# ferreiraluisa/implementation-phd-lab-vision

Hardware: AMD Instinct MI355X
Metric: H36M frames/sec ResNet-50 feature extraction (higher is better)
Workload: dtype bf16; 1 GPU; ResNet-50[:-1] bf16 forward, batch 256 x 224x224x3 fp32 NCHW frames per GPU (BASELINE configs[1]), seeded synthetic weights, (N,2048) fp32 features; batch_per_gpu=256, micro_batch=0, lanes=2, lanes_requested=2, lanes_mode=2 lanes (1.066 x one lane), input=f32, parallelism=frames sharded over 1 rank(s)

## Files before the change

### implementation_phd_lab_vision_amd/csrc/kernels.h

```cpp
#pragma once
#include <hip/hip_runtime.h>
#include <stdint.h>
#include <type_traits>

typedef __attribute__((ext_vector_type(8))) __bf16 bf16x8;
typedef __attribute__((ext_vector_type(4))) float f32x4;
typedef __attribute__((ext_vector_type(4))) unsigned int u32x4;
typedef __attribute__((ext_vector_type(2))) unsigned int u32x2;

#define GLOBAL_AS __attribute__((address_space(1)))
#define LDS_AS __attribute__((address_space(3)))

__device__ __forceinline__ float bf16_bits_to_f32(unsigned int hi16) { return __uint_as_float(hi16 << 16); }

__device__ __forceinline__ unsigned int pack_bf16x2(float lo, float hi) {
    typedef __attribute__((ext_vector_type(2))) __bf16 bf16x2;
    typedef __attribute__((ext_vector_type(2))) float f32x2;
    f32x2 v = {lo, hi};
    bf16x2 b = __builtin_convertvector(v, bf16x2);
    return __builtin_bit_cast(unsigned int, b);
}

typedef __attribute__((ext_vector_type(8))) _Float16 f16x8;
typedef __attribute__((ext_vector_type(2))) _Float16 f16x2;
// ... 561 lines not shown
        unsigned y_voff = 0u;
        constexpr unsigned ESZ = (ET == 2) ? 1u : 2u;
        const unsigned y_rowstep = (unsigned)(16 * a.y_cstride) * ESZ;

        f32x4 bias_reg[MR];
        auto bias_fetch = [&](int tile) {
            const int pt = (int)fast_div((unsigned)tile, a.div_ctiles);
            const int c0 = (tile - pt * a.n_ctiles) * BC;
#pragma unroll
            for (int t = 0; t < MR / 2; ++t) {
                bias_reg[2 * t] = *reinterpret_cast<const f32x4*>(a.bias + c0 + cout_lane + 32 * t);
                bias_reg[2 * t + 1] = *reinterpret_cast<const f32x4*>(a.bias + c0 + cout_lane + 32 * t + 4);
            }
        };
        auto tile_begin = [&]() {
            const int pt = (int)fast_div((unsigned)c_tile, a.div_ctiles);
            const int c0 = (c_tile - pt * a.n_ctiles) * BC, p0 = pt * BP;
            y_voff = (unsigned)((p0 + pix_lane) * a.y_cstride + c0 + cout_lane) * ESZ;
#pragma unroll
            for (int t = 0; t < MR / 2; ++t) {
                const f32x4 b_lo = bias_reg[2 * t];
                const f32x4 b_hi = bias_reg[2 * t + 1];
#pragma unroll
                for (int j = 0; j < NR; ++j) {
                    acc[2 * t][j] = b_lo;
                    acc[2 * t + 1][j] = b_hi;
                    if constexpr (PREFETCH_RES) if (has_res) {
                        if constexpr (ET == 2) {
                            const u32x2 r2 = __builtin_amdgcn_raw_buffer_load_b64(rsrc_r, y_voff + j * y_rowstep + 32 * t, 0, 0);
                            res_reg[t][j] = (u32x4){r2[0], r2[1], 0u, 0u};
                        } else {
                            res_reg[t][j] = __builtin_amdgcn_raw_buffer_load_b128(rsrc_r, y_voff + j * y_rowstep + 64 * t, 0, 0);
                        }
                    }
                }
            }
        };
        auto compute = [&]() {
            const char* sbase = smem + c_buf * STAGE_BYTES;
            bf16x8 wf[2][MR], xf[2][NR];
#pragma unroll
            for (int kk = 0; kk < 2; ++kk) {
                const int ph = fphys0 ^ (kk << 6);
#pragma unroll
                for (int j = 0; j < NR; ++j) xf[kk][j] = *reinterpret_cast<const bf16x8*>(sbase + x_frag + j * 2048 + ph);
#pragma unroll
                for (int m = 0; m < MR; ++m) wf[kk][m] = *reinterpret_cast<const bf16x8*>(sbase + w_frag + m * 2048 + ph);
            }
            if constexpr (ET == 2) {
#pragma unroll
                for (int m = 0; m < MR; ++m)
#pragma unroll
                    for (int j = 0; j < NR; ++j) acc[m][j] = mfma_fp8_k128(wf[0][m], wf[1][m], xf[0][j], xf[1][j], acc[m][j]);
            } else {
#pragma unroll
            for (int kk = 0; kk < 2; ++kk)
#pragma unroll
                for (int m = 0; m < MR; ++m)
#pragma unroll
                    for (int j = 0; j < NR; ++j)
                        acc[m][j] = mfma_e<ET>(wf[kk][m], xf[kk][j], acc[m][j]);
            }
            if constexpr (NCONS + NLOAD <= 8 && ET != 2) {
                __builtin_amdgcn_sched_group_barrier(0x100, 2 * (MR + NR), 0);
                __builtin_amdgcn_sched_group_barrier(0x008, 2 * MR * NR, 0);
            }
        };
        auto epilogue = [&]() {
#pragma unroll
            for (int t = 0; t < MR / 2; ++t) {
#pragma unroll
                for (int j = 0; j < NR; ++j) {
                    f32x4 lo = acc[2 * t][j], hi = acc[2 * t + 1][j];
                    const unsigned voff = y_voff + j * y_rowstep + 32 * ESZ * t;
                    if constexpr (ET == 2) {
#pragma unroll
                        for (int e = 0; e < 4; ++e) { lo[e] *= a.oscale; hi[e] *= a.oscale; }
                        if (has_res) {
                            u32x2 r;
                            if constexpr (PREFETCH_RES) r = (u32x2){res_reg[t][j][0], res_reg[t][j][1]};
                            else r = __builtin_amdgcn_raw_buffer_load_b64(rsrc_r, voff, 0, 0);
                            lo[0] += __builtin_amdgcn_cvt_f32_fp8((int)r[0], 0) * a.rscale; lo[1] += __builtin_amdgcn_cvt_f32_fp8((int)r[0], 1) * a.rscale;
                            lo[2] += __builtin_amdgcn_cvt_f32_fp8((int)r[0], 2) * a.rscale; lo[3] += __builtin_amdgcn_cvt_f32_fp8((int)r[0], 3) * a.rscale;
                            hi[0] += __builtin_amdgcn_cvt_f32_fp8((int)r[1], 0) * a.rscale; hi[1] += __builtin_amdgcn_cvt_f32_fp8((int)r[1], 1) * a.rscale;
                            hi[2] += __builtin_amdgcn_cvt_f32_fp8((int)r[1], 2) * a.rscale; hi[3] += __builtin_amdgcn_cvt_f32_fp8((int)r[1], 3) * a.rscale;
                        }
                        if (a.relu) {
#pragma unroll
                            for (int e = 0; e < 4; ++e) { lo[e] = fmaxf(lo[e], 0.f); hi[e] = fmaxf(hi[e], 0.f); }
                        }
                        const u32x2 o8 = (u32x2){pack4_fp8(lo[0], lo[1], lo[2], lo[3]), pack4_fp8(hi[0], hi[1], hi[2], hi[3])};
                        __builtin_amdgcn_raw_buffer_store_b64(o8, rsrc_y, voff, 0, 0);
                        continue;
                    }
                    if (has_res) {
                        u32x4 r;
                        if constexpr (PREFETCH_RES) r = res_reg[t][j];
                        else r = __builtin_amdgcn_raw_buffer_load_b128(rsrc_r, voff, 0, 0);
                        lo[0] += unpack_lo_e<ET>(r[0]); lo[1] += unpack_hi_e<ET>(r[0]);
                        lo[2] += unpack_lo_e<ET>(r[1]); lo[3] += unpack_hi_e<ET>(r[1]);
                        hi[0] += unpack_lo_e<ET>(r[2]); hi[1] += unpack_hi_e<ET>(r[2]);
                        hi[2] += unpack_lo_e<ET>(r[3]); hi[3] += unpack_hi_e<ET>(r[3]);
                    }
                    u32x4 out = (u32x4){pack2_e<ET>(lo[0], lo[1]), pack2_e<ET>(lo[2], lo[3]), pack2_e<ET>(hi[0], hi[1]),
                                        pack2_e<ET>(hi[2], hi[3])};
                    if (a.relu) {
#pragma unroll
                        for (int e = 0; e < 4; ++e) out[e] = relu_bf16x2(out[e]);
                    }
                    if constexpr (ET != 2) {
                        if (a.q_inv > 0.f) {
                            const u32x2 o8 = (u32x2){
                                pack4_fp8(unpack_lo_e<ET>(out[0]) * a.q_inv, unpack_hi_e<ET>(out[0]) * a.q_inv, unpack_lo_e<ET>(out[1]) * a.q_inv, unpack_hi_e<ET>(out[1]) * a.q_inv),
                                pack4_fp8(unpack_lo_e<ET>(out[2]) * a.q_inv, unpack_hi_e<ET>(out[2]) * a.q_inv, unpack_lo_e<ET>(out[3]) * a.q_inv, unpack_hi_e<ET>(out[3]) * a.q_inv)};
                            __builtin_amdgcn_raw_buffer_store_b64(o8, rsrc_y, voff >> 1, 0, 0);
                            continue;
                        }
                    }
                    __builtin_amdgcn_raw_buffer_store_b128(out, rsrc_y, voff, 0, 0);
                }
            }
        };
        if (total > 0) bias_fetch(c_tile);
        __builtin_amdgcn_s_barrier();
        R50_STAMP_DECL
        for (int g = 0; g < total; ++g) {
            if (c_k == 0) tile_begin();
            R50_MARK(0)
            compute();
#if defined(R50_STAMP)
            __builtin_amdgcn_sched_barrier(0);
            asm volatile("s_nop 0" ::"v"(acc[MR - 1][NR - 1]) : "memory");
#endif
            R50_MARK(1)
            c_buf = (c_buf == NSTAGE - 1) ? 0 : c_buf + 1;
            if (++c_k == a.nk) {
                const int next_tile = c_tile + grid;
                if (next_tile < a.n_blocks) bias_fetch(next_tile);
                epilogue();
                c_k = 0;
                c_tile = next_tile;
            }
            R50_MARK(2)
            __builtin_amdgcn_s_barrier();
            R50_MARK(3)
        }
        R50_STAMP_FLUSH(NCONS + NLOAD)
    }
#else
    (void)a;
#endif
}

template <int ET, int NR, bool DUAL>
__global__ __launch_bounds__(512) void gemm8p_kernel(const ConvArgs a) {
#if defined(__HIP_DEVICE_COMPILE__)
    static_assert(NR == 8 || NR == 7, "pixel blocks per wave: 8 (256-pixel tile) or 7 (224)");
    constexpr int BC = 256, BP = 32 * NR;
    constexpr int NA1 = NR - 4;
    constexpr int SLOT = 16384, KBUF = 4 * SLOT;
    extern __shared__ __attribute__((aligned(16))) char smem[];

    const int tid = threadIdx.x;
    const int lane = tid & 63;
    const int wave = __builtin_amdgcn_readfirstlane(tid >> 6);
    const int wr = wave >> 2, wc = wave & 3;
    const int fr = lane & 15, fq = lane >> 4;
    const int srow = tid >> 3;
    const int lchunk = (tid & 7) ^ (srow & 7);

    const int grid = gridDim.x;
    const int first = xcd_remap(blockIdx.x, grid);
    const int my_tiles = (a.n_blocks - first + grid - 1) / grid;
    const int total = my_tiles * a.nk;

    const __amdgpu_buffer_rsrc_t rsrc_w = __builtin_amdgcn_make_buffer_rsrc(const_cast<__bf16*>(a.w), 0, a.w_bytes, 0x00020000);
    const __amdgpu_buffer_rsrc_t rsrc_x = __builtin_amdgcn_make_buffer_rsrc(const_cast<__bf16*>(a.x), 0, a.x_records, 0x00020000);
    const __amdgpu_buffer_rsrc_t rsrc_x2 = __builtin_amdgcn_make_buffer_rsrc(const_cast<__bf16*>(DUAL ? a.x2 : a.x), 0, DUAL ? a.x2_records : 0u, 0x00020000);
    const __amdgpu_buffer_rsrc_t rsrc_y = __builtin_amdgcn_make_buffer_rsrc(a.y, 0, a.y_bytes, 0x00020000);
    const __amdgpu_buffer_rsrc_t rsrc_r = __builtin_amdgcn_make_buffer_rsrc(const_cast<__bf16*>(a.res), 0, a.res ? a.y_bytes : 0u, 0x00020000);

    unsigned w_voff[2][2], x_voff[2][2], x2_voff[DUAL ? 2 : 1][2];
#pragma unroll
    for (int s = 0; s < 2; ++s)
#pragma unroll
        for (int i = 0; i < 2; ++i) {
            const int q5 = srow & 31;
            const int cl = 128 * i + 64 * (srow >> 5) + 32 * s + ((q5 & 3) | (((q5 >> 4) & 1) << 2) | (((q5 >> 2) & 3) << 3));
            w_voff[s][i] = (unsigned)(cl * a.Ktot + lchunk * 8) * 2u;
        }
    int s_tile = first, s_kt = 0, s_buf = 0, s_rem = total, s_wbase = 0;
    auto decode_tile = [&](int tile) {
        const int pt = (int)fast_div((unsigned)tile, a.div_ctiles);
        const int p0 = pt * BP;
        s_wbase = (tile - pt * a.n_ctiles) * BC * a.Ktot * 2;
#pragma unroll
        for (int s = 0; s < 2; ++s)
#pragma unroll
            for (int i = 0; i < 2; ++i) {
                const int m = p0 + 16 * NR * i + 64 * s + srow;
                unsigned v = kOobOffset, v2 = kOobOffset;
                if ((s == 0 || srow < 16 * NA1) && m < a.M) {
                    const int n = (int)fast_div((unsigned)m, a.div_howo);
                    const int r = m - n * a.HoWo;
                    const int ho = (int)fast_div((unsigned)r, a.div_wo);
                    const int wo = r - ho * a.Wo;
                    v = (unsigned)(((n * a.H + ho * a.stride) * a.W + wo * a.stride) * a.x_cstride + lchunk * 8) * 2u;
                    if constexpr (DUAL) v2 = (unsigned)(((n * a.H2 + ho * a.stride2) * a.W2 + wo * a.stride2) * a.x2_cstride + lchunk * 8) * 2u;
                }
                x_voff[s][i] = v;
                if constexpr (DUAL) x2_voff[s][i] = v2;
            }
    };
    auto stage = [&](auto slot_c) {
        constexpr int SL = decltype(slot_c)::value;
        if (s_rem > 0) {
            char* dst = smem + s_buf * KBUF + SL * SLOT + wave * 1024;
            if constexpr ((SL & 1) == 0) {
                const int soff = __builtin_amdgcn_readfirstlane(s_wbase + s_kt * 128);
#pragma unroll
                for (int i = 0; i < 2; ++i)
                    __builtin_amdgcn_raw_ptr_buffer_load_lds(rsrc_w, (LDS_AS void*)(dst + i * 8192), 16, w_voff[SL >> 1][i], soff, 0, 0);
            } else {
                const bool second = DUAL && s_kt >= a.cc1;
                const int soff = __builtin_amdgcn_readfirstlane((second ? s_kt - a.cc1 : s_kt) * 128);
                const __amdgpu_buffer_rsrc_t rs = second ? rsrc_x2 : rsrc_x;
#pragma unroll
                for (int i = 0; i < 2; ++i) {
                    const unsigned v = second ? x2_voff[DUAL ? (SL >> 1) : 0][i] : x_voff[SL >> 1][i];
                    __builtin_amdgcn_raw_ptr_buffer_load_lds(rs, (LDS_AS void*)(dst + i * 8192), 16, v, soff, 0, 0);
                }
            }
            if constexpr (SL == 3) {
                --s_rem;
                s_buf ^= 1;
                if (++s_kt == a.nk) {
                    s_kt = 0;
                    s_tile += grid;
                    if (s_tile < a.n_blocks) decode_tile(s_tile);
                }
            }
        }
    };
    using std::integral_constant;

    f32x4 acc[4][NR];
    f32x4 bias_reg[4];
    const bool has_res = (a.res != nullptr);
    const int fphys0 = (fq ^ (fr & 7)) << 4;
    const int w_fr[2] = {(32 * wc + fr) * 128 + fphys0, (32 * wc + fr) * 128 + (fphys0 ^ 64)};
    const int x_fr[2] = {SLOT + (64 * wr + fr) * 128 + fphys0, SLOT + (64 * wr + fr) * 128 + (fphys0 ^ 64)};
    const int cout_lane = 64 * wc + 8 * fq;
    const int pix_lane = 16 * NR * wr + fr;
    int c_tile = first, c_kt = 0;
    unsigned y_voff = 0u;
    const unsigned y_rowstep = (unsigned)(16 * a.y_cstride * 2);
    auto bias_fetch = [&](int tile) {
        const int pt = (int)fast_div((unsigned)tile, a.div_ctiles);
        const int c0 = (tile - pt * a.n_ctiles) * BC;
#pragma unroll
        for (int t = 0; t < 2; ++t) {
            bias_reg[2 * t] = *reinterpret_cast<const f32x4*>(a.bias + c0 + cout_lane + 32 * t);
            bias_reg[2 * t + 1] = *reinterpret_cast<const f32x4*>(a.bias + c0 + cout_lane + 32 * t + 4);
        }
    };
    auto tile_begin = [&]() {
        const int pt = (int)fast_div((unsigned)c_tile, a.div_ctiles);
        const int c0 = (c_tile - pt * a.n_ctiles) * BC, p0 = pt * BP;
        y_voff = (unsigned)((p0 + pix_lane) * a.y_cstride + c0 + cout_lane) * 2u;
#pragma unroll
        for (int m = 0; m < 4; ++m)
#pragma unroll
            for (int j = 0; j < NR; ++j) acc[m][j] = bias_reg[m];
    };
    auto epilogue = [&]() {
#pragma unroll
        for (int j = 0; j < NR; ++j) {
            u32x4 rres[2];
            if (has_res) {
#pragma unroll
                for (int t = 0; t < 2; ++t) rres[t] = __builtin_amdgcn_raw_buffer_load_b128(rsrc_r, y_voff + j * y_rowstep + 64 * t, 0, 0);
            }
#pragma unroll
            for (int t = 0; t < 2; ++t) {
                f32x4 lo = acc[2 * t][j], hi = acc[2 * t + 1][j];
                if (has_res) {
                    const u32x4 r = rres[t];
                    lo[0] += unpack_lo_e<ET>(r[0]); lo[1] += unpack_hi_e<ET>(r[0]);
                    lo[2] += unpack_lo_e<ET>(r[1]); lo[3] += unpack_hi_e<ET>(r[1]);
                    hi[0] += unpack_lo_e<ET>(r[2]); hi[1] += unpack_hi_e<ET>(r[2]);
                    hi[2] += unpack_lo_e<ET>(r[3]); hi[3] += unpack_hi_e<ET>(r[3]);
                }
                u32x4 out = (u32x4){pack2_e<ET>(lo[0], lo[1]), pack2_e<ET>(lo[2], lo[3]), pack2_e<ET>(hi[0], hi[1]), pack2_e<ET>(hi[2], hi[3])};
                if (a.relu) {
#pragma unroll
                    for (int e = 0; e < 4; ++e) out[e] = relu_bf16x2(out[e]);
                }
                __builtin_amdgcn_raw_buffer_store_b128(out, rsrc_y, y_voff + j * y_rowstep + 64 * t, 0, 0);
            }
        }
    };
#define G8_BARRIER() { __builtin_amdgcn_sched_barrier(0); __builtin_amdgcn_s_barrier(); __builtin_amdgcn_sched_barrier(0); }
#define G8_LGKM(n) { asm volatile("s_waitcnt lgkmcnt(" #n ")" ::: "memory"); __builtin_amdgcn_sched_barrier(0); }
#define G8_PRIO_UP() __builtin_amdgcn_s_setprio(1)
#define G8_PRIO_DN() __builtin_amdgcn_s_setprio(0)

    if (total > 0) {
        bias_fetch(c_tile);
        decode_tile(s_tile);
        stage(integral_constant<int, 0>{}); stage(integral_constant<int, 1>{}); stage(integral_constant<int, 2>{}); stage(integral_constant<int, 3>{});
        stage(integral_constant<int, 0>{}); stage(integral_constant<int, 1>{}); stage(integral_constant<int, 2>{});
        if (total >= 2) {
            asm volatile("s_waitcnt vmcnt(6)" ::: "memory");
        } else {
            asm volatile("s_waitcnt vmcnt(0)" ::: "memory");
        }
    }
    G8_BARRIER();
    if (wr == 1) G8_BARRIER();

    bf16x8 xf[4][2], wf0[2][2], wf1[2][2];
    for (int g = 0; g < total; ++g) {
        const char* kb = smem + (g & 1) * KBUF;
        if (c_kt == 0) tile_begin();
#pragma unroll
        for (int m = 0; m < 2; ++m)
#pragma unroll
            for (int kk = 0; kk < 2; ++kk) wf0[m][kk] = *reinterpret_cast<const bf16x8*>(kb + w_fr[kk] + m * 2048);
        __builtin_amdgcn_sched_barrier(0);
#pragma unroll
        for (int j = 0; j < 4; ++j)
#pragma unroll
            for (int kk = 0; kk < 2; ++kk) xf[j][kk] = *reinterpret_cast<const bf16x8*>(kb + x_fr[kk] + j * 2048);
        __builtin_amdgcn_sched_barrier(0);
        stage(integral_constant<int, 3>{});
        G8_LGKM(8)
        G8_BARRIER();
        G8_LGKM(0)
        G8_PRIO_UP();
#pragma unroll
        for (int kk = 0; kk < 2; ++kk)
#pragma unroll
            for (int m = 0; m < 2; ++m)
#pragma unroll
                for (int j = 0; j < 4; ++j) acc[m][j] = mfma_e<ET>(wf0[m][kk], xf[j][kk], acc[m][j]);
        G8_PRIO_DN();
        G8_BARRIER();
#pragma unroll
        for (int m = 0; m < 2; ++m)
#pragma unroll
            for (int kk = 0; kk < 2; ++kk) wf1[m][kk] = *reinterpret_cast<const bf16x8*>(kb + 2 * SLOT + w_fr[kk] + m * 2048);
        __builtin_amdgcn_sched_barrier(0);
        stage(integral_constant<int, 0>{});
        G8_BARRIER();
        G8_LGKM(0)
        G8_PRIO_UP();
#pragma unroll
        for (int kk = 0; kk < 2; ++kk)
#pragma unroll
            for (int m = 0; m < 2; ++m)
#pragma unroll
                for (int j = 0; j < 4; ++j) acc[2 + m][j] = mfma_e<ET>(wf1[m][kk], xf[j][kk], acc[2 + m][j]);
        G8_PRIO_DN();
        G8_BARRIER();
#pragma unroll
        for (int j = 0; j < NA1; ++j)
#pragma unroll
            for (int kk = 0; kk < 2; ++kk) xf[j][kk] = *reinterpret_cast<const bf16x8*>(kb + 2 * SLOT + x_fr[kk] + j * 2048);
        __builtin_amdgcn_sched_barrier(0);
        stage(integral_constant<int, 1>{});
        G8_BARRIER();
        G8_LGKM(0)
        G8_PRIO_UP();
#pragma unroll
        for (int kk = 0; kk < 2; ++kk)
#pragma unroll
            for (int m = 0; m < 2; ++m)
#pragma unroll
                for (int j = 0; j < NA1; ++j) acc[2 + m][4 + j] = mfma_e<ET>(wf1[m][kk], xf[j][kk], acc[2 + m][4 + j]);
        G8_PRIO_DN();
        G8_BARRIER();
        stage(integral_constant<int, 2>{});
        if (g + 2 < total) {
            asm volatile("s_waitcnt vmcnt(6)" ::: "memory");
        } else {
            asm volatile("s_waitcnt vmcnt(0)" ::: "memory");
        }
        G8_BARRIER();
        G8_PRIO_UP();
#pragma unroll
        for (int kk = 0; kk < 2; ++kk)
#pragma unroll
            for (int m = 0; m < 2; ++m)
#pragma unroll
                for (int j = 0; j < NA1; ++j) acc[m][4 + j] = mfma_e<ET>(wf0[m][kk], xf[j][kk], acc[m][4 + j]);
        G8_PRIO_DN();
        G8_BARRIER();
        if (++c_kt == a.nk) {
            const int next_tile = c_tile + grid;
            if (next_tile < a.n_blocks) bias_fetch(next_tile);
            epilogue();
            c_kt = 0;
            c_tile = next_tile;
        }
    }
    if (wr == 0) G8_BARRIER();
#undef G8_BARRIER
#undef G8_LGKM
#undef G8_PRIO_UP
#undef G8_PRIO_DN
#else
    (void)a;
#endif
}

template <int ET>
__global__ __launch_bounds__(512) void conv3x3_c64_kernel(const ConvArgs a) {
#if defined(__HIP_DEVICE_COMPILE__)
    constexpr int W_BYTES = 9 * 64 * 128;
    constexpr int XROWS_LDS = 352;
    constexpr int X_BYTES = XROWS_LDS * 128;
    constexpr int NPASS = 11;
    extern __shared__ __attribute__((aligned(16))) char smem[];
    const int tid = threadIdx.x, lane = tid & 63;
    const int wave = __builtin_amdgcn_readfirstlane(tid >> 6);

    for (int i = tid; i < 9 * 64 * 8; i += 512) {
        const int c = i & 7, rho = (i >> 3) & 63, tap = i >> 9;
        const int cl = (rho & ~31) | (rho & 3) | (((rho >> 4) & 1) << 2) | (((rho >> 2) & 3) << 3);
        *reinterpret_cast<u32x4*>(smem + tap * 8192 + rho * 128 + ((c ^ (rho & 7)) << 4)) =
            *reinterpret_cast<const u32x4*>(a.w + (size_t)cl * 576 + tap * 64 + c * 8);
    }
    const int grid = gridDim.x;
    const int n_tiles = a.N * 14;
    const int first = blockIdx.x;
    const int my_tiles = (n_tiles - first + grid - 1) / grid;

    if (wave >= 4) {
        const int lw = wave - 4;
        const __amdgpu_buffer_rsrc_t rsrc_x = __builtin_amdgcn_make_buffer_rsrc(
            const_cast<char*>(reinterpret_cast<const char*>(a.x) - a.x_back), 0, a.x_records, 0x00020000);
        unsigned rel[NPASS];
        unsigned top_mask = 0u, bot_mask = 0u, ok_mask = 0u;
#pragma unroll
        for (int i = 0; i < NPASS; ++i) {
            const int rho = i * 32 + lw * 8 + (lane >> 3);
            const int rr = rho / 58, col = rho - rr * 58;
            const int chunk = (lane & 7) ^ (col & 7);
            rel[i] = (unsigned)((rr * 56 + col) * 128 + chunk * 16);
            if (rho < 348 && col >= 1 && col <= 56) ok_mask |= 1u << i;
            if (rr == 0) top_mask |= 1u << i;
            if (rr == 5) bot_mask |= 1u << i;
        }
        auto issue = [&](int tile, int buf) {
            const int n = tile / 14, tr = tile - n * 14;
            const unsigned base = (unsigned)((n * 56 + tr * 4) * 56) * 128u;
            unsigned valid = ok_mask;
            if (tr == 0) valid &= ~top_mask;
            if (tr == 13) valid &= ~bot_mask;
            char* dst = smem + W_BYTES + buf * X_BYTES + lw * 1024;
#pragma unroll
            for (int i = 0; i < NPASS; ++i) {
                const unsigned voff = ((valid >> i) & 1u) ? base + rel[i] : kOobOffset;
                __builtin_amdgcn_raw_ptr_buffer_load_lds(rsrc_x, (LDS_AS void*)(dst + i * 4096), 16, voff, 0, 0, 0);
            }
        };
        if (my_tiles > 0) issue(first, 0);
        __syncthreads();
        for (int t = 0; t < my_tiles; ++t) {
            asm volatile("s_waitcnt vmcnt(0)" ::: "memory");
            __builtin_amdgcn_s_barrier();
            if (t + 1 < my_tiles) issue(first + (t + 1) * grid, (t + 1) & 1);
        }
    } else {
        const int wave_c = wave >> 1, wave_p = wave & 1;
        const int fr = lane & 15, fq = lane >> 4;
        const __amdgpu_buffer_rsrc_t rsrc_y = __builtin_amdgcn_make_buffer_rsrc(a.y, 0, a.y_bytes, 0x00020000);
        const int cout_lane = wave_c * 32 + 8 * fq;
        const f32x4 b_lo = *reinterpret_cast<const f32x4*>(a.bias + cout_lane);
        const f32x4 b_hi = *reinterpret_cast<const f32x4*>(a.bias + cout_lane + 4);
        const int w_frag = (wave_c * 32 + fr) * 128 + ((fq ^ (fr & 7)) << 4);
        int xa[7][3];
#pragma unroll
        for (int j = 0; j < 7; ++j) {
            const int p = wave_p * 112 + 16 * j + fr;
            const int r = p / 56, c = p - r * 56;
#pragma unroll
            for (int kw = 0; kw < 3; ++kw) xa[j][kw] = (r * 58 + c + kw) * 128 + ((fq ^ ((c + kw) & 7)) << 4);
        }
        __syncthreads();
        for (int t = 0; t < my_tiles; ++t) {
            __builtin_amdgcn_s_barrier();
            const char* xb = smem + W_BYTES + (t & 1) * X_BYTES;
            f32x4 acc[2][7];
#pragma unroll
            for (int j = 0; j < 7; ++j) { acc[0][j] = b_lo; acc[1][j] = b_hi; }
            bf16x8 wf[2][2], xf[2][7];
            auto read_block = [&](int it, bf16x8 (&w)[2], bf16x8 (&x)[7]) {
                const int tap = it >> 1, kk = it & 1, kh = tap / 3, kw = tap - kh * 3;
                const char* wt = smem + tap * 8192;
                w[0] = *reinterpret_cast<const bf16x8*>(wt + (w_frag ^ (kk << 6)));
                w[1] = *reinterpret_cast<const bf16x8*>(wt + 2048 + (w_frag ^ (kk << 6)));
#pragma unroll
                for (int j = 0; j < 7; ++j)
                    x[j] = *reinterpret_cast<const bf16x8*>(xb + kh * (58 * 128) + (xa[j][kw] ^ (kk << 6)));
            };
            read_block(0, wf[0], xf[0]);
#pragma unroll
            for (int it = 0; it < 18; ++it) {
                if (it + 1 < 18) read_block(it + 1, wf[(it + 1) & 1], xf[(it + 1) & 1]);
#pragma unroll
                for (int j = 0; j < 7; ++j) {
                    acc[0][j] = mfma_e<ET>(wf[it & 1][0], xf[it & 1][j], acc[0][j]);
                    acc[1][j] = mfma_e<ET>(wf[it & 1][1], xf[it & 1][j], acc[1][j]);
                }
                if (it + 1 < 18) __builtin_amdgcn_sched_group_barrier(0x100, 9, 0);
                __builtin_amdgcn_sched_group_barrier(0x008, 14, 0);
            }
            const int tile = first + t * grid;
            const unsigned pix0 = (unsigned)(tile * 224 + wave_p * 112 + fr);
#pragma unroll
            for (int j = 0; j < 7; ++j) {
                const f32x4 lo = acc[0][j], hi = acc[1][j];
                u32x4 o = (u32x4){pack2_e<ET>(lo[0], lo[1]), pack2_e<ET>(lo[2], lo[3]), pack2_e<ET>(hi[0], hi[1]),
                                  pack2_e<ET>(hi[2], hi[3])};
                if (a.relu) {
#pragma unroll
                    for (int e = 0; e < 4; ++e) o[e] = relu_bf16x2(o[e]);
                }
                __builtin_amdgcn_raw_buffer_store_b128(o, rsrc_y, (pix0 + 16 * j) * 128u + cout_lane * 2, 0, 0);
            }
        }
    }
#else
    (void)a;
#endif
}

template <int ET, int NI, int TR, int IW, int IH>
__global__ __launch_bounds__(768) void conv3x3_xres_kernel(const ConvArgs a) {
#if defined(__HIP_DEVICE_COMPILE__)
    constexpr int BC = 128, TPS = 1, NST = 3, SCHED = 0, RB = 1;
    constexpr bool RB7 = RB && IW == 7;
    static_assert(RB == 0 || (TPS == 1 && (NST == 3 || RB == 1) && SCHED == 0 && ((NI == 1 && (IW == 14 || IW == 28) && TR * (IW == 14 ? 16 : 32) == 224) || (NI == 4 && IW == 7 && TR == 7 && RB == 1))),
                  "row blocks: 14 blocks of 16 positions");
    static_assert(RB != 3 || BC == 128, "32-wide blocks: four consumer waves of 32 couts");
    constexpr int NCW = RB == 3 ? 4 : 8;
    constexpr int PW = RB ? (IW == 28 ? 32 : 16) : IW + 2, PP = (TR + 2) * PW, PPT = RB7 ? 17 * 16 : NI * PP;
    constexpr int BSTEP = RB7 ? 8 : 7;
    constexpr int XPASS = (PPT + 31) / 32, XBUF = XPASS * 32 * 128;
    constexpr int NPX = NI * TR * IW, NBLK = RB ? 14 : (NPX + 15) / 16;
    static_assert(RB || NBLK == 13, "tiles are 196 pixels");
// ... 4981 lines not shown
```

### implementation_phd_lab_vision_amd/csrc/r50_abi.hip

```cpp
#include "kernels.h"
#include "smooth_kernels.h"
#include "multiview_kernels.h"
#include "kinematics_kernels.h"
#include "refine_kernels.h"
#include "track_kernels.h"
#include "resample_kernels.h"
#include "bootstrap_kernels.h"
#include "launch_plan.h"
#include "../../include/r50.h"
#include "../../include/r50_hal.h"
#include "../../include/r50_smooth.h"
#include "../../include/r50_multiview.h"
#include "../../include/r50_kinematics.h"
#include "../../include/r50_refine.h"
#include "../../include/r50_track.h"
#include "../../include/r50_resample.h"
#include "../../include/r50_bootstrap.h"

#include <atomic>
#include <cmath>
#include <cstdlib>
#include <cstdio>
#include <cstring>
#include <initializer_list>
// ... 294 lines not shown
                    out[(((size_t)kh * 64 + rho) * 8 + (kw + 1)) * 4 + c] = part == 2 ? f32_to_f16_rne(w) : part ? f32_to_bf16_rne(w - bf16_to_f32(hd)) : hd;
                }
        }
}

FastDiv make_fast_div(unsigned d) {
    FastDiv f{0u, 0u};
    if (d <= 1u) return f;
    unsigned L = 0;
    while ((1ull << L) < d) ++L;
    f.shr = L - 1;
    const unsigned long long num = 1ull << (32 + f.shr);
    f.mul = (unsigned)((num + d - 1) / d);
    return f;
}

constexpr int kPersistBit = 32;
int g_num_cus = 0;
int g_cu_cap = [] { const char* v = std::getenv("R50_CU_CAP"); return v ? std::atoi(v) : 0; }();
int cu_budget(int device_cus) { return (g_cu_cap > 0 && g_cu_cap < device_cus) ? g_cu_cap : device_cus; }
int num_cus() {
    if (g_num_cus == 0) {
        int dev = 0;
        hipDeviceProp_t prop;
        if (hipGetDevice(&dev) != hipSuccess || hipGetDeviceProperties(&prop, dev) != hipSuccess) return 0;
        g_num_cus = cu_budget(prop.multiProcessorCount);
    }
    return g_num_cus;
}

template <typename K, typename... Args>
Launch launch_persistent(K kern, long long tiles, int threads, size_t lds, hipStream_t s, Args... args) {
    const hipError_t e = hipFuncSetAttribute(reinterpret_cast<const void*>(kern), hipFuncAttributeMaxDynamicSharedMemorySize, (int)lds);
    if (e != hipSuccess) return e;
    const int cus = num_cus();
    if (cus == 0) return hipErrorInvalidDevice;
    hipLaunchKernelGGL(kern, dim3((unsigned)(tiles < cus ? tiles : cus)), dim3(threads), lds, s, args...);
    return hipGetLastError();
}

template <int ET, int BC, int BP, int WC, int WP, int NSTAGE, bool SPLIT = false>
Launch launch_igemm_t(ConvArgs a, bool persistent, hipStream_t s) {
    a.n_ctiles = a.Cout / BC;
    a.n_blocks = a.n_ctiles * ((a.M + BP - 1) / BP);
    a.div_ctiles = make_fast_div((unsigned)a.n_ctiles);
    constexpr int kRowsPerPass = WC * WP * 8;
    const size_t lds = (size_t)NSTAGE * (BC + (BP + kRowsPerPass - 1) / kRowsPerPass * kRowsPerPass) * 128;
    auto kern = igemm_bf16_kernel<ET, BC, BP, WC, WP, NSTAGE, SPLIT>;
    if (lds > 65536) {
        hipError_t e = hipFuncSetAttribute(reinterpret_cast<const void*>(kern),
                                           hipFuncAttributeMaxDynamicSharedMemorySize, (int)lds);
        if (e != hipSuccess) return e;
    }
    int grid = a.n_blocks;
    if (persistent) {
        const int cus = num_cus();
        if (cus == 0) return hipErrorInvalidDevice;
        static int per_cu = 0;
        if (per_cu == 0) {
            int n = 0;
            if (hipOccupancyMaxActiveBlocksPerMultiprocessor(&n, kern, WC * WP * 64, lds) != hipSuccess || n < 1) n = 1;
            per_cu = n;
        }
        if (grid > cus * per_cu) grid = cus * per_cu;
    }
    hipLaunchKernelGGL(kern, dim3(grid), dim3(WC * WP * 64), lds, s, a);
    return hipGetLastError();
}

struct TunedTile { int h, cin, cout, ks, stride, res, tile; };
constexpr TunedTile kTuned[] = {
    {56, 64, 64, 1, 1, 0, 73},    {56, 64, 64, 3, 1, 0, 2},     {56, 64, 256, 1, 1, 1, 72},   {56, 64, 256, 1, 1, 0, 38},
    {56, 256, 64, 1, 1, 0, 73},    {56, 256, 128, 1, 1, 0, 40},  {56, 128, 128, 3, 2, 0, 65},   {28, 128, 512, 1, 1, 1, 72},
    {56, 256, 512, 1, 2, 0, 42},  {28, 512, 128, 1, 1, 0, 65},   {28, 128, 128, 3, 1, 0, 72},  {28, 512, 256, 1, 1, 0, 72},
    {28, 256, 256, 3, 2, 0, 44},  {14, 256, 1024, 1, 1, 1, 72}, {28, 512, 1024, 1, 2, 0, 72}, {14, 1024, 256, 1, 1, 0, 44},
    {14, 256, 256, 3, 1, 0, 68},  {14, 1024, 512, 1, 1, 0, 72}, {14, 512, 512, 3, 2, 0, 68},  {7, 512, 2048, 1, 1, 1, 43},
    {14, 1024, 2048, 1, 2, 0, 43}, {7, 2048, 512, 1, 1, 0, 72}, {7, 512, 512, 3, 1, 0, 68},
};

constexpr int kWsBit = 64;

template <int ET, int BC, int BP, int CWC, int CWP, int NLOAD, int NSTAGE>
Launch launch_igemm_ws_t(ConvArgs a, hipStream_t s) {
    a.n_ctiles = a.Cout / BC;
    a.n_blocks = a.n_ctiles * ((a.M + BP - 1) / BP);
    a.div_ctiles = make_fast_div((unsigned)a.n_ctiles);
    constexpr int kRowsPerPass = NLOAD * 8;
    const size_t lds = (size_t)NSTAGE * (BC + (BP + kRowsPerPass - 1) / kRowsPerPass * kRowsPerPass) * 128;
    return launch_persistent(igemm_ws_kernel<ET, BC, BP, CWC, CWP, NLOAD, NSTAGE>, a.n_blocks, (CWC * CWP + NLOAD) * 64, lds, s, a);
}

constexpr int kTileC64 = kWsBit | 16;
bool is_c64_shape(const ConvArgs& a) {
    return a.ks == 3 && a.stride == 1 && a.pad == 1 && a.Cin == 64 && a.Cout == 64 && a.H == 56 && a.W == 56 && a.res == nullptr &&
           a.x_cstride == 64 && a.y_cstride == 64 && a.Ktot == 576;
}
template <int ET>
Launch launch_conv3x3_c64(const ConvArgs& a, hipStream_t s) {
    if (!is_c64_shape(a)) return Launch::refused();
    constexpr size_t lds = 9 * 64 * 128 + 2 * 352 * 128;
    return launch_persistent(conv3x3_c64_kernel<ET>, a.N * 14, 512, lds, s, a);
}

constexpr int kTileXres = kWsBit | 17;
bool is_xres_shape(const ConvArgs& a) {
    if (!(a.ks == 3 && a.stride == 1 && a.pad == 1 && a.Cin == a.Cout && a.H == a.W && a.res == nullptr && a.x2 == nullptr &&
          a.x_cstride == a.Cin && a.y_cstride == a.Cout && a.Ktot == 9 * a.Cin && a.et != 2)) return false;
    return (a.H == 14 && a.Cin == 256) || (a.H == 7 && a.Cin == 512) || (a.H == 28 && a.Cin == 128);
}
template <int ET, int NI, int TR, int IW, int IH>
Launch launch_conv3x3_xres_t(ConvArgs a, hipStream_t s) {
    constexpr int BC = 128, NST = 3;
    constexpr int PW = IW == 28 ? 32 : 16;
    constexpr int PPT = IW == 7 ? 17 * 16 : NI * (TR + 2) * PW, XBUF = (PPT + 31) / 32 * 32 * 128;
    constexpr size_t lds = 2 * (size_t)XBUF + NST * (size_t)BC * 128;
    static_assert(lds <= 163840, "LDS budget");
    a.n_ctiles = a.Cout / BC;
    a.n_blocks = ((a.N + NI - 1) / NI) * (IH / TR) * a.n_ctiles;
    return launch_persistent(conv3x3_xres_kernel<ET, NI, TR, IW, IH>, a.n_blocks, 768, lds, s, a);
}
template <int ET>
Launch launch_conv3x3_xres(const ConvArgs& a, hipStream_t s) {
    if (!is_xres_shape(a)) return Launch::refused();
    if (a.H == 14) return launch_conv3x3_xres_t<ET, 1, 14, 14, 14>(a, s);
    if (a.H == 28) return launch_conv3x3_xres_t<ET, 1, 7, 28, 28>(a, s);
    return launch_conv3x3_xres_t<ET, 4, 7, 7, 7>(a, s);
}

constexpr int kTileS2 = kWsBit | 18;
bool is_s2_shape(const ConvArgs& a) {
    if (!(a.ks == 3 && a.stride == 2 && a.pad == 1 && a.Cin == a.Cout && a.H == a.W && a.res == nullptr && a.x2 == nullptr &&
          a.x_cstride == a.Cin && a.y_cstride == a.Cout && a.Ktot == 9 * a.Cin && a.et != 2)) return false;
    return (a.H == 56 && a.Cin == 128) || (a.H == 28 && a.Cin == 256) || (a.H == 14 && a.Cin == 512);
}
template <int ET, int TR, int OW, int OH>
Launch launch_conv3x3_s2_t(ConvArgs a, hipStream_t s) {
    constexpr size_t lds = 3 * 32768 + 3 * 128 * 128;
    a.n_ctiles = a.Cout / 128;
    a.n_blocks = (OW == 7 ? (a.N + 3) / 4 : a.N * (OH / TR)) * a.n_ctiles;
    return launch_persistent(conv3x3_s2_kernel<ET, 128, TR, OW, OH>, a.n_blocks, 768, lds, s, a);
}
template <int ET>
Launch launch_conv3x3_s2(const ConvArgs& a, hipStream_t s) {
    if (!is_s2_shape(a)) return Launch::refused();
    if (a.H == 56) return launch_conv3x3_s2_t<ET, 7, 28, 28>(a, s);
    if (a.H == 14) return launch_conv3x3_s2_t<ET, 7, 7, 7>(a, s);
    return launch_conv3x3_s2_t<ET, 14, 14, 14>(a, s);
}

constexpr int kTileG8 = kWsBit | 19;
constexpr int kTileG8N7 = kWsBit | 20;
bool is_g8_shape(const ConvArgs& a) {
    return a.ks == 1 && a.pad == 0 && a.Cout % 256 == 0 && a.et != 2 && a.x_wrap >= (1 << 30) && a.q_inv == 0.f &&
           a.y_cstride == a.Cout && a.nk >= 1 && (a.x2 ? (a.stride == 1 && a.cc1 >= 1 && a.cc1 < a.nk) : a.x_cstride == a.Cin);
}
template <int ET, int NR, bool DUAL>
Launch launch_gemm8p_t(ConvArgs a, hipStream_t s) {
    constexpr int BP = 32 * NR;
    constexpr size_t lds = 2 * 4 * 16384;
    a.n_ctiles = a.Cout / 256;
    a.n_blocks = a.n_ctiles * ((a.M + BP - 1) / BP);
    a.div_ctiles = make_fast_div((unsigned)a.n_ctiles);
    return launch_persistent(gemm8p_kernel<ET, NR, DUAL>, a.n_blocks, 512, lds, s, a);
}
template <int ET>
Launch launch_gemm8p(const ConvArgs& a, int tile, hipStream_t s) {
    if (!is_g8_shape(a)) return Launch::refused();
    if (a.x2) return tile == kTileG8N7 ? launch_gemm8p_t<ET, 7, true>(a, s) : launch_gemm8p_t<ET, 8, true>(a, s);
    return tile == kTileG8N7 ? launch_gemm8p_t<ET, 7, false>(a, s) : launch_gemm8p_t<ET, 8, false>(a, s);
}

long long tiles_of(const ConvArgs& a, int tile) {
    int bc = 0, bp = 0;
    if (tile & kWsBit) {
        switch (tile & (kPersistBit - 1)) {
            case 1: bc = 128; bp = 128; break;  case 3: bc = 256; bp = 128; break;  case 4: case 8: bc = 128; bp = 224; break;
            case 9: bc = 64; bp = 224; break;   case 10: bc = 128; bp = 208; break;   case 19: bc = 256; bp = 256; break;   case 20: bc = 256; bp = 224; break;
            default: return 0;
        }
    } else {
        switch (tile & (kPersistBit - 1)) {
            case 1: case 8: bc = 128; bp = 128; break;  case 2: bc = 64; bp = 128; break;   case 3: bc = 64; bp = 256; break;
            case 5: bc = 128; bp = 64; break;           case 6: bc = 256; bp = 128; break;  case 7: bc = 128; bp = 256; break;
            case 9: case 10: bc = 256; bp = 256; break; case 11: bc = 256; bp = 208; break; case 12: bc = 256; bp = 224; break;
            default: return 0;
        }
    }
    if (a.Cout % bc) return 0;
    return (long long)(a.Cout / bc) * ((a.M + bp - 1) / bp);
}

int g_use_xres = [] { const char* v = std::getenv("R50_XRES"); return v ? std::atoi(v) : 1; }();
int g_use_s2 = [] { const char* v = std::getenv("R50_S2"); return v ? std::atoi(v) : 1; }();
int g_use_g8 = [] { const char* v = std::getenv("R50_G8"); return v ? std::atoi(v) : 1; }();
struct G8Shape { int h, cin, cout, two_sources; };
constexpr G8Shape kG8[] = {{14, 1024, 256, 0}, {14, 1024, 512, 0}, {14, 768, 1024, 1}, {7, 1536, 2048, 1}};
int g8_tile(const ConvArgs& a) {
    if (!g_use_g8 || !is_g8_shape(a) || a.N < 48) return 0;
    if (g_use_g8 == 2) return kTileG8;
    if (g_use_g8 == 3) return kTileG8N7;
    for (const G8Shape& g : kG8)
        if (g.h == a.Ho && a.Ho == a.Wo && g.cin == a.Ktot && g.cout == a.Cout && (g.two_sources != 0) == (a.x2 != nullptr) && a.stride == 1 && !a.res)
            return tiles_of(a, kTileG8N7) >= 200 ? kTileG8N7 : 0;
    return 0;
}
int auto_tile(const ConvArgs& a) {
    if (is_c64_shape(a)) return kTileC64;
    if (const int t8 = g8_tile(a)) return t8;
    if (g_use_xres && is_xres_shape(a)) return kTileXres;
    if (g_use_s2 && is_s2_shape(a)) return kTileS2;
    const long long want = 200;
    if (a.N >= 48 && a.H == a.W)
        for (const TunedTile& t : kTuned)
            if (t.h == a.H && t.cin == a.Cin && t.cout == a.Cout && t.ks == a.ks && t.stride == a.stride &&
                t.res == (a.res != nullptr)) {
                if (tiles_of(a, t.tile) >= want) return t.tile;
                break;
            }
    const int cand[] = {kWsBit | 8, 1, 5, 2};
    int best = 2;
    long long best_n = -1;
    for (int c : cand) {
        const long long n = tiles_of(a, c);
        if (n >= want) return c;
        if (n > best_n) { best_n = n; best = c; }
    }
    return best;
}

template <int ET>
Launch launch_igemm_et(const ConvArgs& a, int tile, hipStream_t s, bool split) {
    if (split && ET != 0) return Launch::refused();
    if (split) {
        if (a.Cout % 128) return launch_igemm_t<0, 64, 128, 1, 4, 2, true>(a, false, s);
        return launch_igemm_t<0, 128, 128, 2, 2, 2, true>(a, false, s);
    }
    if (tile == 0) tile = auto_tile(a);
    if (a.x2 && (!(tile & kWsBit) || tile == kTileC64 || tile == kTileXres || tile == kTileS2)) return Launch::refused();
    if (tile == kTileG8 || tile == kTileG8N7) return launch_gemm8p<ET>(a, tile, s);
    const bool pers = (tile & kPersistBit) != 0;
    if (tile == kTileC64) return launch_conv3x3_c64<ET>(a, s);
    if (tile == kTileXres) return launch_conv3x3_xres<ET>(a, s);
    if (tile == kTileS2) return launch_conv3x3_s2<ET>(a, s);
    if (tile & kWsBit) {
        switch (tile & (kPersistBit - 1)) {
            case 1: if (a.Cout % 128) return Launch::refused(); return launch_igemm_ws_t<ET, 128, 128, 2, 2, 4, 4>(a, s);
            case 3: if (a.Cout % 256) return Launch::refused(); return launch_igemm_ws_t<ET, 256, 128, 4, 2, 4, 3>(a, s);
            case 4: if (a.Cout % 128) return Launch::refused(); return launch_igemm_ws_t<ET, 128, 224, 2, 2, 4, 3>(a, s);
            case 8: if (a.Cout % 128) return Launch::refused(); return launch_igemm_ws_t<ET, 128, 224, 4, 2, 4, 3>(a, s);
            case 9: return launch_igemm_ws_t<ET, 64, 224, 2, 2, 4, 4>(a, s);
            case 10: if (a.Cout % 128) return Launch::refused(); return launch_igemm_ws_t<ET, 128, 208, 4, 1, 4, 3>(a, s);
            default: return Launch::refused();
        }
    }
    switch (tile & (kPersistBit - 1)) {
        case 1: if (a.Cout % 128) return Launch::refused(); return launch_igemm_t<ET, 128, 128, 2, 2, 2>(a, pers, s);
        case 2: return launch_igemm_t<ET, 64, 128, 1, 4, 2>(a, pers, s);
        case 3: return launch_igemm_t<ET, 64, 256, 1, 4, 2>(a, pers, s);
        case 5: if (a.Cout % 128) return Launch::refused(); return launch_igemm_t<ET, 128, 64, 2, 2, 2>(a, pers, s);
        case 6: if (a.Cout % 256) return Launch::refused(); return launch_igemm_t<ET, 256, 128, 4, 2, 3>(a, pers, s);
        case 7: if (a.Cout % 128) return Launch::refused(); return launch_igemm_t<ET, 128, 256, 2, 4, 3>(a, pers, s);
        case 8: if (a.Cout % 128) return Launch::refused(); return launch_igemm_t<ET, 128, 128, 2, 4, 3>(a, pers, s);
        case 9: if (a.Cout % 256) return Launch::refused(); return launch_igemm_t<ET, 256, 256, 4, 2, 2>(a, pers, s);
        case 10: if (a.Cout % 256) return Launch::refused(); return launch_igemm_t<ET, 256, 256, 2, 4, 2>(a, pers, s);
        case 11: if (a.Cout % 256) return Launch::refused(); return launch_igemm_t<ET, 256, 208, 8, 1, 2>(a, pers, s);
        case 12: if (a.Cout % 256) return Launch::refused(); return launch_igemm_t<ET, 256, 224, 4, 2, 2>(a, pers, s);
        default: return Launch::refused();
    }
}

Launch launch_igemm(const ConvArgs& a, int tile, hipStream_t s, bool split = false) {
    return R50_BY_ET(a.et, launch_igemm_et)(a, tile, s, split);
}

Launch launch_igemm_fp8(const ConvArgs& a, int tile, hipStream_t s) {
    if (tile == 0) {
        tile = kWsBit | 9;
        for (int c : {kWsBit | 8, kWsBit | 3, kWsBit | 1})
            if (tiles_of(a, c) >= 200) { tile = c; break; }
    }
    if (!(tile & kWsBit) || tile == kTileC64) return Launch::refused();
    switch (tile & (kPersistBit - 1)) {
        case 1: if (a.Cout % 128) return Launch::refused(); return launch_igemm_ws_t<2, 128, 128, 2, 2, 4, 4>(a, s);
        case 3: if (a.Cout % 256) return Launch::refused(); return launch_igemm_ws_t<2, 256, 128, 4, 2, 4, 3>(a, s);
        case 4: if (a.Cout % 128) return Launch::refused(); return launch_igemm_ws_t<2, 128, 224, 2, 2, 4, 3>(a, s);
        case 8: if (a.Cout % 128) return Launch::refused(); return launch_igemm_ws_t<2, 128, 224, 4, 2, 4, 3>(a, s);
        case 9: return launch_igemm_ws_t<2, 64, 224, 2, 2, 4, 4>(a, s);
        default: return Launch::refused();
    }
}

Launch fill_conv_args(ConvArgs& a, const void* x, int n, int h, int w, int cin, const void* wt, const float* bias,
                      const void* res, void* y, int cout, int ks, int stride, int pad, int relu, bool split = false, bool w2 = false) {
    Launch r;
    if (!x || !wt || !bias || !y) return Launch::refused();
    if (n <= 0 || h <= 0 || w <= 0 || cin <= 0 || cin % 64 || cout <= 0 || cout % 64) return Launch::refused();
    if (!(ks == 1 || ks == 3) || stride < 1 || pad < 0 || 2 * pad > ks - 1) return Launch::refused();
    a.x = (const __bf16*)x; a.w = (const __bf16*)wt; a.bias = bias; a.res = (const __bf16*)res; a.y = (__bf16*)y;
    a.N = n; a.H = h; a.W = w; a.Cin = cin; a.Cout = cout;
    a.Ho = (h + 2 * pad - ks) / stride + 1;
    a.Wo = (w + 2 * pad - ks) / stride + 1;
    if (a.Ho <= 0 || a.Wo <= 0) return Launch::refused();
    a.ks = ks; a.stride = stride; a.pad = pad; a.relu = relu;
    const long long M = (long long)n * a.Ho * a.Wo;
    if (size_over(r, "output pixels n*ho*wo", M, (1ll << 30) + 1, "2^30 + 1")) return r;
    a.M = (int)M; a.HoWo = a.Ho * a.Wo;
    a.x_cstride = split ? 2 * cin : cin;
    a.y_cstride = split ? 2 * cout : cout;
    const int kmul = split ? 3 : (w2 ? 2 : 1);
    a.x_wrap = split ? 2 * (cin / 64) : (w2 ? cin / 64 : (1 << 30));
    a.cin_chunks = kmul * (cin / 64); a.nk = ks * ks * a.cin_chunks; a.Ktot = ks * ks * kmul * cin;
    a.n_ctiles = 0; a.n_blocks = 0;
    const long long x_bytes = (long long)n * h * w * a.x_cstride * 2;
    const long long x_back = ((long long)pad * w + pad) * a.x_cstride * 2;
    if (size_over(r, "x bytes + back reach, n*h*w*cx*2 + (pad*w+pad)*cx*2 (cx = channels per x pixel),", x_bytes + x_back, k2p31, "2^31") ||
        size_over(r, "w bytes, cout*K*2 (K = weight elements per cout),", (long long)cout * ks * ks * kmul * cin * 2, k2p31, "2^31") ||
        size_over(r, "y bytes, n*ho*wo*cy*2 (cy = channels per y pixel),", M * a.y_cstride * 2, k2p31, "2^31"))
        return r;
    a.x_back = (int)x_back;
    a.x_records = (unsigned)(x_bytes + a.x_back);
    a.w_bytes = (unsigned)((long long)cout * a.Ktot * 2);
    a.y_bytes = (unsigned)(M * a.y_cstride * 2);
    a.div_howo = make_fast_div((unsigned)a.HoWo);
    a.div_wo = make_fast_div((unsigned)a.Wo);
    a.div_ctiles = FastDiv{0u, 0u};
    a.et = 0;
    a.oscale = 1.0f; a.rscale = 1.0f; a.q_inv = 0.0f;
    a.x2 = nullptr; a.H2 = 0; a.W2 = 0; a.stride2 = 1; a.x2_cstride = 0; a.cc1 = 1 << 30; a.x2_records = 0u;
#if defined(R50_STAMP)
    a.dbg = nullptr;
#endif
    return r;
}

void prof_begin(r50_handle* h, hipStream_t s, EvRec& r, int cls, double flops, double bytes, int layer = -1) {
    if (!h || !h->profile) return;
    r.layer = layer;
    auto get = [&]() {
        hipEvent_t e;
        if (!h->ev_free.empty()) { e = h->ev_free.back(); h->ev_free.pop_back(); }
        else (void)hipEventCreate(&e);
        return e;
    };
    r.a = get(); r.b = get(); r.cls = cls; r.flops = flops; r.bytes = bytes;
    (void)hipEventRecord(r.a, s);
}
void prof_end(r50_handle* h, hipStream_t s, EvRec& r) {
    if (!h || !h->profile) return;
    (void)hipEventRecord(r.b, s);
    h->ev_pending.push_back(r);
}
const std::string kNoKey;
template <typename F>
int profiled(r50_handle* h, hipStream_t s, int cls, double flops, double bytes, int layer, const char* what, const std::string& key, F&& launch,
             const char* key_suffix = "") {
// ... 2325 lines not shown
```

Before: 103,300 frames/s.

## Route layer4 residual 1x1 conv to gemm8p with early-prefetched residual loads

Adds a compile-time RES variant of the persistent gemm8p kernel and routes the 7x7 512->2048 residual 1x1 convolution to it instead of the previous tile choice. On the last K step of each tile, part of the residual rows are loaded with inline-asm buffer loads ahead of time. The rest are loaded just before the epilogue, with vmcnt waits adjusted so those loads overlap the final MMA work rather than stalling the epilogue. This costs extra VGPRs to hold the residual fragments, which may lower occupancy or cause spills, and the hand-tuned wait counts are fragile.

```diff
diff --git a/implementation_phd_lab_vision_amd/csrc/kernels.h b/implementation_phd_lab_vision_amd/csrc/kernels.h
--- a/implementation_phd_lab_vision_amd/csrc/kernels.h
+++ b/implementation_phd_lab_vision_amd/csrc/kernels.h
@@ -737,10 +737,11 @@
 #endif
 }
 
-template <int ET, int NR, bool DUAL>
+template <int ET, int NR, bool DUAL, bool RES = false>
 __global__ __launch_bounds__(512) void gemm8p_kernel(const ConvArgs a) {
 #if defined(__HIP_DEVICE_COMPILE__)
     static_assert(NR == 8 || NR == 7, "pixel blocks per wave: 8 (256-pixel tile) or 7 (224)");
+    static_assert(!(DUAL && RES), "the two-source form has no identity add (the network never has both)");
     constexpr int BC = 256, BP = 32 * NR;
     constexpr int NA1 = NR - 4;
     constexpr int SLOT = 16384, KBUF = 4 * SLOT;
@@ -831,7 +832,8 @@
 
     f32x4 acc[4][NR];
     f32x4 bias_reg[4];
-    const bool has_res = (a.res != nullptr);
+    constexpr int NPF = RES ? (NR == 7 ? 4 : 2) : 0;
+    u32x4 rres[RES ? NR : 1][2];
     const int fphys0 = (fq ^ (fr & 7)) << 4;
     const int w_fr[2] = {(32 * wc + fr) * 128 + fphys0, (32 * wc + fr) * 128 + (fphys0 ^ 64)};
     const int x_fr[2] = {SLOT + (64 * wr + fr) * 128 + fphys0, SLOT + (64 * wr + fr) * 128 + (fphys0 ^ 64)};
@@ -858,19 +860,36 @@
 #pragma unroll
             for (int j = 0; j < NR; ++j) acc[m][j] = bias_reg[m];
     };
+    const u32x4 rdesc_r = (u32x4){(unsigned)(uintptr_t)a.res, (unsigned)((uintptr_t)a.res >> 32), RES ? a.y_bytes : 0u, 0x00020000u};
+    auto res_fetch_early = [&]() {
+#pragma unroll
+        for (int j = 0; j < NPF; ++j) {
+            const unsigned v = y_voff + j * y_rowstep;
+            asm volatile("buffer_load_dwordx4 %0, %1, %2, 0 offen" : "=&v"(rres[j][0]) : "v"(v), "s"(rdesc_r) : "memory");
+            asm volatile("buffer_load_dwordx4 %0, %1, %2, 0 offen offset:64" : "=&v"(rres[j][1]) : "v"(v), "s"(rdesc_r) : "memory");
+        }
+    };
+    auto res_land = [&]() {
+#pragma unroll
+        for (int j = NPF; j < (RES ? NR : 0); ++j)
+#pragma unroll
+            for (int t = 0; t < 2; ++t) rres[j][t] = __builtin_amdgcn_raw_buffer_load_b128(rsrc_r, y_voff + j * y_rowstep + 64 * t, 0, 0);
+        __builtin_amdgcn_sched_barrier(0);
+        asm volatile("s_waitcnt vmcnt(%0)" ::"n"(4 + 2 * (NR - NPF)) : "memory");
+#pragma unroll
+        for (int j = 0; j < NPF; ++j)
+#pragma unroll
+            for (int t = 0; t < 2; ++t) asm volatile("" : "+v"(rres[j][t]));
+        __builtin_amdgcn_sched_barrier(0);
+    };
     auto epilogue = [&]() {
 #pragma unroll
         for (int j = 0; j < NR; ++j) {
-            u32x4 rres[2];
-            if (has_res) {
-#pragma unroll
-                for (int t = 0; t < 2; ++t) rres[t] = __builtin_amdgcn_raw_buffer_load_b128(rsrc_r, y_voff + j * y_rowstep + 64 * t, 0, 0);
-            }
 #pragma unroll
             for (int t = 0; t < 2; ++t) {
                 f32x4 lo = acc[2 * t][j], hi = acc[2 * t + 1][j];
-                if (has_res) {
-                    const u32x4 r = rres[t];
+                if constexpr (RES) {
+                    const u32x4 r = rres[j][t];
                     lo[0] += unpack_lo_e<ET>(r[0]); lo[1] += unpack_hi_e<ET>(r[0]);
                     lo[2] += unpack_lo_e<ET>(r[1]); lo[3] += unpack_hi_e<ET>(r[1]);
                     hi[0] += unpack_lo_e<ET>(r[2]); hi[1] += unpack_hi_e<ET>(r[2]);
@@ -908,6 +927,7 @@
     for (int g = 0; g < total; ++g) {
         const char* kb = smem + (g & 1) * KBUF;
         if (c_kt == 0) tile_begin();
+        const bool last = RES && c_kt == a.nk - 1;
 #pragma unroll
         for (int m = 0; m < 2; ++m)
 #pragma unroll
@@ -937,6 +957,10 @@
             for (int kk = 0; kk < 2; ++kk) wf1[m][kk] = *reinterpret_cast<const bf16x8*>(kb + 2 * SLOT + w_fr[kk] + m * 2048);
         __builtin_amdgcn_sched_barrier(0);
         stage(integral_constant<int, 0>{});
+        if constexpr (RES) {
+            if (last) res_fetch_early();
+            __builtin_amdgcn_sched_barrier(0);
+        }
         G8_BARRIER();
         G8_LGKM(0)
         G8_PRIO_UP();
@@ -967,7 +991,11 @@
         G8_BARRIER();
         stage(integral_constant<int, 2>{});
         if (g + 2 < total) {
-            asm volatile("s_waitcnt vmcnt(6)" ::: "memory");
+            if (last) {
+                asm volatile("s_waitcnt vmcnt(%0)" ::"n"(6 + 2 * NPF) : "memory");
+            } else {
+                asm volatile("s_waitcnt vmcnt(6)" ::: "memory");
+            }
         } else {
             asm volatile("s_waitcnt vmcnt(0)" ::: "memory");
         }
@@ -983,6 +1011,7 @@
         G8_BARRIER();
         if (++c_kt == a.nk) {
             const int next_tile = c_tile + grid;
+            if constexpr (RES) res_land();
             if (next_tile < a.n_blocks) bias_fetch(next_tile);
             epilogue();
             c_kt = 0;
diff --git a/implementation_phd_lab_vision_amd/csrc/r50_abi.hip b/implementation_phd_lab_vision_amd/csrc/r50_abi.hip
--- a/implementation_phd_lab_vision_amd/csrc/r50_abi.hip
+++ b/implementation_phd_lab_vision_amd/csrc/r50_abi.hip
@@ -470,21 +470,22 @@
 constexpr int kTileG8N7 = kWsBit | 20;
 bool is_g8_shape(const ConvArgs& a) {
     return a.ks == 1 && a.pad == 0 && a.Cout % 256 == 0 && a.et != 2 && a.x_wrap >= (1 << 30) && a.q_inv == 0.f &&
-           a.y_cstride == a.Cout && a.nk >= 1 && (a.x2 ? (a.stride == 1 && a.cc1 >= 1 && a.cc1 < a.nk) : a.x_cstride == a.Cin);
-}
-template <int ET, int NR, bool DUAL>
+           a.y_cstride == a.Cout && a.nk >= 1 && (a.x2 ? (a.stride == 1 && a.cc1 >= 1 && a.cc1 < a.nk && !a.res) : a.x_cstride == a.Cin);
+}
+template <int ET, int NR, bool DUAL, bool RES = false>
 Launch launch_gemm8p_t(ConvArgs a, hipStream_t s) {
     constexpr int BP = 32 * NR;
     constexpr size_t lds = 2 * 4 * 16384;
     a.n_ctiles = a.Cout / 256;
     a.n_blocks = a.n_ctiles * ((a.M + BP - 1) / BP);
     a.div_ctiles = make_fast_div((unsigned)a.n_ctiles);
-    return launch_persistent(gemm8p_kernel<ET, NR, DUAL>, a.n_blocks, 512, lds, s, a);
+    return launch_persistent(gemm8p_kernel<ET, NR, DUAL, RES>, a.n_blocks, 512, lds, s, a);
 }
 template <int ET>
 Launch launch_gemm8p(const ConvArgs& a, int tile, hipStream_t s) {
     if (!is_g8_shape(a)) return Launch::refused();
     if (a.x2) return tile == kTileG8N7 ? launch_gemm8p_t<ET, 7, true>(a, s) : launch_gemm8p_t<ET, 8, true>(a, s);
+    if (a.res) return tile == kTileG8N7 ? launch_gemm8p_t<ET, 7, false, true>(a, s) : launch_gemm8p_t<ET, 8, false, true>(a, s);
     return tile == kTileG8N7 ? launch_gemm8p_t<ET, 7, false>(a, s) : launch_gemm8p_t<ET, 8, false>(a, s);
 }
 
@@ -511,14 +512,15 @@
 int g_use_xres = [] { const char* v = std::getenv("R50_XRES"); return v ? std::atoi(v) : 1; }();
 int g_use_s2 = [] { const char* v = std::getenv("R50_S2"); return v ? std::atoi(v) : 1; }();
 int g_use_g8 = [] { const char* v = std::getenv("R50_G8"); return v ? std::atoi(v) : 1; }();
-struct G8Shape { int h, cin, cout, two_sources; };
-constexpr G8Shape kG8[] = {{14, 1024, 256, 0}, {14, 1024, 512, 0}, {14, 768, 1024, 1}, {7, 1536, 2048, 1}};
+struct G8Shape { int h, cin, cout, two_sources, res; };
+constexpr G8Shape kG8[] = {{14, 1024, 256, 0, 0}, {14, 1024, 512, 0, 0}, {14, 768, 1024, 1, 0}, {7, 1536, 2048, 1, 0}, {7, 512, 2048, 0, 1}};
 int g8_tile(const ConvArgs& a) {
     if (!g_use_g8 || !is_g8_shape(a) || a.N < 48) return 0;
     if (g_use_g8 == 2) return kTileG8;
     if (g_use_g8 == 3) return kTileG8N7;
     for (const G8Shape& g : kG8)
-        if (g.h == a.Ho && a.Ho == a.Wo && g.cin == a.Ktot && g.cout == a.Cout && (g.two_sources != 0) == (a.x2 != nullptr) && a.stride == 1 && !a.res)
+        if (g.h == a.Ho && a.Ho == a.Wo && g.cin == a.Ktot && g.cout == a.Cout && (g.two_sources != 0) == (a.x2 != nullptr) && a.stride == 1 &&
+            (g.res != 0) == (a.res != nullptr))
             return tiles_of(a, kTileG8N7) >= 200 ? kTileG8N7 : 0;
     return 0;
 }
```

After: 103,300 frames/s (median of 2 runs). About the same (+0.1%).
